# RichealYoung/BRIEF_PyTorch

Hardware: AMD Instinct MI355X
Metric: encode_voxels_per_sec (higher is better)
Workload: dtype f32; 1 GPU; SingleTask 512^3 synthetic uint16 volume, SIREN 4x256 (layers=5, features=256, w0=20), randompoint sample_size=100000, datal2, Adamax lr=1e-3; layers=5, features=256, sample_size=100000, params=198657

## Files before the change

__graft_entry__.py:

```python
import os
import subprocess
import sys

ROOT = os.path.dirname(os.path.abspath(__file__))
if ROOT not in sys.path:
    sys.path.insert(0, ROOT)


def build():
    from brief_pytorch_amd import _lib
    _lib.build(verbose=True)
    subprocess.check_call(["make", "-s", "-C", os.path.join(ROOT, "oracle")])
    import brief_pytorch_amd
    L = _lib.lib()
    for name in _lib.EXPORTS:
        assert hasattr(L, name), name
    print("build ok: libbrief_hip.so version", L.brief_version())


def smoke():
    import numpy as np
    import torch
    from brief_pytorch_amd import _lib
    from brief_pytorch_amd.networks import SIREN
    from brief_pytorch_amd.synthetic import make_volume
    from oracle import oracle as O

    assert torch.cuda.is_available(), "smoke() needs a GPU"
    _lib.lib()
    dims = (12, 16, 20)
    vol = make_volume(dims, seed=1)
    vn, side = O.normalize(vol)
    n = int(np.prod(dims))
    tv = torch.from_numpy(vn.reshape(-1, 1)).cuda()
    for layers, feats in ((5, 256), (4, 64), (3, 1100)):
        torch.manual_seed(0)
        m = SIREN(coords_channel=3, data_channel=1, features=feats, layers=layers, w0=20)
        d = O.make_desc(3, 1, layers, feats, 20.0)
        p = m.params.numpy().copy()
        m.to("cuda")
        loss, _ = m.train_step(n, tv, grid=(dims, -1.0, 1.0))
        lo, go, _, _ = O.loss_grad(d, p, O.grid_coords(dims), vn.reshape(-1, 1))
        g = m.grads.cpu().numpy()
        assert abs(loss.item() - lo) / lo < 1e-5, (loss.item(), lo)
# ... 12 lines not shown
```

brief_pytorch_amd/_lib.py:

```python
import ctypes as C
import os
import subprocess

_HERE = os.path.dirname(os.path.abspath(__file__))
LIB_PATH = os.environ.get("BRIEF_LIB", os.path.join(_HERE, "libbrief_hip.so"))
SRC = os.path.join(_HERE, "csrc", "brief_hip.hip")
_CSRC = os.path.join(_HERE, "csrc")
_DEPS = sorted(os.path.join(_CSRC, f) for f in (os.listdir(_CSRC) if os.path.isdir(_CSRC) else []) if f.endswith((".hip", ".inc", ".h"))) \
    + [os.path.join(os.path.dirname(_HERE), "include", "brief_hip.h")]
HIPCC = os.environ.get("HIPCC", "/opt/rocm/bin/hipcc")


class BriefError(RuntimeError):
    pass


class SirenDesc(C.Structure):
    _fields_ = [("cin", C.c_int32), ("cout", C.c_int32), ("layers", C.c_int32), ("features", C.c_int32),
                ("w0_first", C.c_float), ("w0_hidden", C.c_float), ("output_act", C.c_int32), ("precision", C.c_int32)]


class GridDesc(C.Structure):
    _fields_ = [("ndim", C.c_int32), ("reserved", C.c_int32), ("dims", C.c_int64 * 3), ("lo", C.c_float), ("hi", C.c_float)]

# ... 68 lines not shown

class TaperDesc(C.Structure):
    _fields_ = [("cin", C.c_int32), ("cout", C.c_int32), ("layers", C.c_int32), ("output_act", C.c_int32),
                ("widths", C.c_int32 * TAPER_MAX_LAYERS), ("w0", C.c_float * TAPER_MAX_LAYERS)]


class TaperFitJob(C.Structure):
    _fields_ = [("desc", TaperDesc)] + FitJob._fields_[1:]


FAMILIES = (("ffn", FfnDesc, FfnFitJob), ("nerf", NerfDesc, NerfFitJob), ("mfn", MfnDesc, MfnFitJob), ("taper", TaperDesc, TaperFitJob))
FAMILY_ENTRIES = ("param_count", "packed_count", "train_workspace_bytes", "repack", "forward", "forward_box", "train_step", "fit")

LOSS_KIND = {"datal2": 0, "datasmoothl1": 1, "external": 2}
OPT_KIND = {"Adamax": 0, "Adam": 1, "SGD": 2}
OUT_F32, OUT_U8, OUT_U16 = 0, 1, 2
PRECISION = {"fp32": 0, "f32": 0, "bf16": 1, "bf16x3": 2}

EXPORTS = ["brief_version", "brief_last_error", "brief_param_count", "brief_packed_count",
           "brief_train_workspace_bytes", "brief_siren_repack", "brief_siren_forward", "brief_forward_workspace_bytes", "brief_siren_forward_ws", "brief_siren_forward_box", "brief_siren_train_step", "brief_siren_fit_step",
           "brief_siren_fit", "brief_multi_fit",
           "brief_optim_step", "brief_sample_indices", "brief_sse_u16", "brief_profile_enable", "brief_profile_fused", "brief_deblock_edge", "brief_ssim_u16", "brief_ssim_partial_count",
           "brief_sincos_probe", "brief_cu_count",
           "brief_correct_chunk_elems", "brief_correct_count", "brief_correct_emit", "brief_correct_apply",
           "brief_mip_accumulate",
           "brief_quant_workspace_bytes", "brief_quant_ranges", "brief_quant_apply", "brief_quant_decode",
           "brief_siren_jac_packed_count", "brief_siren_jac_repack", "brief_siren_jac_forward", "brief_siren_jac_forward_box",
           "brief_view_clip", "brief_view_coords", "brief_view_fold", "brief_view_finish", "brief_view_sample_host", "brief_view_clip_host",
           "brief_surface_fold", "brief_surface_bracket", "brief_surface_coords", "brief_surface_step", "brief_surface_shade",
           "brief_view_sample_t_host"] \
    + ["brief_%s_%s" % (prefix, entry) for prefix, _, _ in FAMILIES for entry in FAMILY_ENTRIES]


def needs_build():
    if LIB_PATH != os.path.join(_HERE, "libbrief_hip.so"):
        return False
    if not os.path.exists(LIB_PATH):
        return True
    t = os.path.getmtime(LIB_PATH)
    return any(os.path.exists(d) and os.path.getmtime(d) > t for d in _DEPS)


DIAG_LIB_PATH = os.path.join(_HERE, "libbrief_hip_diag.so")


def build(force=False, verbose=False, diagnostics=False, defines=(), out=None):
    target = out or (DIAG_LIB_PATH if diagnostics else os.path.join(_HERE, "libbrief_hip.so"))
    if not force and not diagnostics and not defines and out is None and not needs_build():
        return LIB_PATH
    cmd = [HIPCC, "--offload-arch=gfx950", "-O3", "-std=c++17", "-ffp-contract=off", "-shared", "-fPIC", SRC, "-o", target]
    if diagnostics:
        cmd.append("-DBRIEF_DIAGNOSTICS")
    cmd += ["-D" + d for d in defines]
    if verbose:
        print(" ".join(cmd))
    subprocess.check_call(cmd)
    return target


_LIB = None


def lib():
    global _LIB
    if _LIB is not None:
        return _LIB
    import torch
    if not os.path.exists(LIB_PATH):
        raise BriefError("libbrief_hip.so is not built (run `python -c 'import __graft_entry__ as g; g.build()'`); "
                         "there is no CPU fallback for the fused SIREN path")
    L = C.CDLL(LIB_PATH)
    dp, gp, bp, vp = C.POINTER(SirenDesc), C.POINTER(GridDesc), C.POINTER(BatchDesc), C.c_void_p
    L.brief_version.restype = C.c_int
    if L.brief_version() != 130:
        raise BriefError("libbrief_hip.so is version %d, this binding needs 130 (brief_siren_forward_ws, widths to 4096): rebuild with __graft_entry__.build()" % L.brief_version())
    L.brief_last_error.restype = C.c_char_p
    L.brief_param_count.restype = C.c_int64
    L.brief_param_count.argtypes = [dp]
    L.brief_packed_count.restype = C.c_int64
    L.brief_packed_count.argtypes = [dp]
    L.brief_train_workspace_bytes.restype = C.c_int64
    L.brief_train_workspace_bytes.argtypes = [dp, C.c_int64]
# ... 83 lines not shown
```

brief_pytorch_amd/csrc/brief_hip.hip:

```cpp
#include <hip/hip_runtime.h>
#include <hip/hip_ext.h>
#include <stdint.h>
#include <stdio.h>
#include <string.h>
#include <stdlib.h>
#include <mutex>
#include "brief_layout.h"
#include "brief_math.h"

#include "brief_device.inc"
#include "brief_fused.inc"
#include "brief_lean.inc"
#include "brief_wide.inc"
#include "brief_small.inc"
#include "brief_wgrad.inc"
#include "brief_x3.inc"
#include "brief_reduce.inc"
#include "brief_bf16.inc"
#include "brief_aux.inc"
#include "brief_ffn.inc"
#include "brief_nerf.inc"
#include "brief_mfn.inc"
#include "brief_taper.inc"
#include "brief_correct.inc"
#include "brief_mip.inc"
#include "brief_quant.inc"
#include "brief_jac.inc"

static thread_local char g_err[512] = "";
static int fail(int code, const char *fmt, const char *detail = "")
{
    snprintf(g_err, sizeof(g_err), fmt, detail);
    return code;
}
#define HIP_TRY(x)                                                                  \
    do {                                                                            \
        hipError_t e_ = (x);                                                        \
        if (e_ != hipSuccess) return fail(BRIEF_ERR_LAUNCH, #x ": %s", hipGetErrorString(e_)); \
    } while (0)
// ... 46 lines not shown
static DevState *dev_state()
{
    std::lock_guard<std::recursive_mutex> lk(g_state_mu);
    static DevState *tab[kMaxDevices] = {};
    const int dev = current_device();
    if (!tab[dev]) tab[dev] = (DevState *)calloc(1, sizeof(DevState));
    return tab[dev];
}
static int dev_attr_once(const void *fn, int bytes)
{
    std::lock_guard<std::recursive_mutex> lk(g_state_mu);
    DevState *ds = dev_state();
    if (!ds) return fail(BRIEF_ERR_INVALID, "out of host memory");
    for (int i = 0; i < ds->nattr; ++i)
        if (ds->attr_fn[i] == fn && ds->attr_bytes[i] >= bytes) return 0;
    HIP_TRY(hipFuncSetAttribute(fn, hipFuncAttributeMaxDynamicSharedMemorySize, bytes));
    if (ds->nattr < 256) { ds->attr_fn[ds->nattr] = fn; ds->attr_bytes[ds->nattr] = bytes; ++ds->nattr; }
    return 0;
}

static int cu_count()
{
    static int cached[64] = {};
    int dev = 0;
    if (hipGetDevice(&dev) != hipSuccess || dev < 0 || dev >= 64) dev = 0;
    if (cached[dev] == 0) {
        int n = 0;
        if (hipDeviceGetAttribute(&n, hipDeviceAttributeMultiprocessorCount, dev) != hipSuccess || n < 1) n = 256;
        cached[dev] = n;
    }
    return cached[dev];
}
#define kCUs cu_count()
#define kWgradBlocks cu_count()

static OptimScalars optim_scalars(int kind, double lr, double beta1, double beta2, double eps, int64_t t)
{
    OptimScalars o;
    o.kind = kind;
    o.w1 = (float)(1.0 - beta1); o.fb2 = (float)beta2; o.w2 = (float)(1.0 - beta2); o.feps = (float)eps;
    o.nstep = kind == BRIEF_OPT_SGD ? (float)(-lr) : (float)(-(lr / (1.0 - pow(beta1, (double)t))));
    o.bc2s = kind == BRIEF_OPT_ADAM ? (float)sqrt(1.0 - pow(beta2, (double)t)) : 1.f;
    return o;
}

#ifdef BRIEF_DIAGNOSTICS
static const char *env_str(const char *name) { return getenv(name); }
#else
static const char *env_str(const char *) { return nullptr; }
#endif
static int env_int(const char *name, int dflt, int lo, int hi)
{
    const char *e = env_str(name);
    if (!e) return dflt;
    const int v = atoi(e);
    return v >= lo && v <= hi ? v : dflt;
}
static const int kRecWgsPerCu = 8;
static const int g_wg_per_cu = env_int("BRIEF_WG_PER_CU", BRIEF_TRAIN_WPE, 1, 4);
static const bool g_wg_per_cu_set = env_str("BRIEF_WG_PER_CU") != nullptr;
static const int g_stagger = env_int("BRIEF_STAGGER", 0, 0, 64);
static const int g_diag = env_int("BRIEF_DIAG", 0, 0, 255);
static const int g_x3_decode = env_int("BRIEF_X3_DECODE", 1, 0, 1);
static const int g_wgrad_repeat = env_int("BRIEF_WGRAD_REPEAT", 1, 1, 8);
static const int g_reduce_sg_big = env_int("BRIEF_REDUCE_SG_BIG", 4, 1, 64);
static const int g_reduce_part = env_int("BRIEF_REDUCE_PART", 0, 0, 2);
// ... 31 lines not shown
    const int64_t wgs_ = fused_wg_samples(d, train);
    const int64_t tiles = (n + wgs_ - 1) / wgs_;
    const int cap = fused_grid(d, n, train);
    FusedPlan p;
    p.grid = cap; p.pers_wgs = cap; p.pers_tiles = tiles;
    if (!train || nt > 8 || tiles <= cap || brief_use_wide(d)) return p;
    if (g_tail_rounds == 0) return p;
    int64_t rounds = tiles / cap - g_tail_rounds;
    if (rounds < 0) rounds = 0;
    const int64_t max_wgs = (int64_t)kCUs * kRecWgsPerCu;
    while (tiles - rounds * cap + (rounds ? cap : 0) > max_wgs) ++rounds;
    if (rounds * cap >= tiles) return p;
    p.pers_wgs = rounds ? cap : 0;
    p.pers_tiles = rounds * cap;
    p.grid = p.pers_wgs + (int)(tiles - p.pers_tiles);
    return p;
}
#ifndef BRIEF_WGRAD_ROUNDS
#define BRIEF_WGRAD_ROUNDS 1
#endif
#ifndef BRIEF_TAIL_PLAN
#define BRIEF_TAIL_PLAN 1
#endif
#ifndef BRIEF_TAIL_LEAN
#define BRIEF_TAIL_LEAN 0
#endif
#ifndef BRIEF_TAIL_MODE_DEFAULT
#define BRIEF_TAIL_MODE_DEFAULT 2
#endif
#ifndef BRIEF_TAIL_R
#define BRIEF_TAIL_R 1.15
#define BRIEF_TAIL_R1 1.05
#endif
#ifndef BRIEF_TAIL_MIN_SPLITS
#define BRIEF_TAIL_MIN_SPLITS 6
#endif
#ifndef BRIEF_TAIL_MIN_ROUNDS
#define BRIEF_TAIL_MIN_ROUNDS 3
#endif
struct TailPlan { int mode ; bool on; int grid_body, grid_tail; int64_t tiles_body; int ns, n_norm; int64_t kfix_n, kfix_s; };
static int wgrad_split_rule(const brief_siren_desc &d, int64_t nchunks, int min_rounds);
static const int g_tail_mode = env_int("BRIEF_TAIL_MODE", BRIEF_TAIL_MODE_DEFAULT, 0, 2);
static const int g_tail_ntmax = env_int("BRIEF_TAIL_NTMAX", 32, 9, 32);
static const int g_tail_r = env_int("BRIEF_TAIL_R", 0, 0, 1000);
static TailPlan fused_tail_plan(const brief_siren_desc &d, int64_t n)
{
    TailPlan p;
    memset(&p, 0, sizeof(p));
    if (!BRIEF_TAIL_PLAN || g_tail_mode == 0 || d.precision != BRIEF_PREC_F32 || d.layers - 2 < 1) return p;
    const int nt = brief_nt(d);
    if (nt < 8) return p;
    const int64_t tiles = (n + 31) / 32;
    const int G = fused_grid(d, n, true);
    const int64_t full = tiles / G * G, rem = tiles - full;
    if (full == 0 || rem == 0) return p;
    if (g_tail_mode == 2 && nt >= 9 && nt <= g_tail_ntmax && rem * 4 <= 3 * (int64_t)kCUs) {
        const int hidden = d.layers - 2, nq = wgrad_nq(nt), qt = (nt + nq - 1) / nq;
        const int64_t chunks = brief_npad_d(d, n) / 32, B = (int64_t)hidden * nq * nq;
        int ns = wgrad_split_rule(d, chunks, 1);
        if ((int64_t)ns * B > kCUs) ns = (int)(kCUs / B);
        const int per_xcd = kCUs / 8, tail_x = (int)((rem + 7) / 8);
        int n_norm = 0;
        if ((int64_t)ns * B <= kCUs)
            for (int c = ns - 1; c >= 1; --c) {
                const int a_ = (int)((c * B + 7) / 8), s_ = (int)(((ns - c) * B + 7) / 8);
                if (a_ + tail_x <= per_xcd && a_ + s_ <= per_xcd && (ns - c) * B >= rem) { n_norm = c; break; }
            }
        const int n_short = ns - n_norm;
        const double r = g_tail_r ? 0.01 * g_tail_r : (nt <= 16 ? BRIEF_TAIL_R : BRIEF_TAIL_R1);
        const double rho = r * 2.0 * hidden * nt * nt / (double)(qt * qt);
        const double k_norm = ((double)chunks + n_short * rho) / ns, k_short = k_norm - rho;
        if (n_norm > 0 && k_short >= 4.0 && rho < 0.8 * k_norm) {
            p.kfix_n = (int64_t)(k_norm * 65536.0); p.kfix_s = (int64_t)(k_short * 65536.0);
            const int64_t b_norm = ((int64_t)(ns - n_short) * p.kfix_n) >> 16;
            if (b_norm <= full && b_norm > 0) {
                p.mode = 2; p.on = true; p.grid_body = G; p.grid_tail = (int)rem; p.tiles_body = full; p.ns = ns; p.n_norm = ns - n_short;
                return p;
            }
        }
    }
    if (!(brief_use_wide(d) || (BRIEF_TAIL_LEAN && brief_use_lean(d, true) && nt >= 9))) return p;
    if (rem * 4 > 3 * (int64_t)G) return p;
    if (wgrad_split_rule(d, full, BRIEF_TAIL_MIN_ROUNDS) < BRIEF_TAIL_MIN_SPLITS) return p;
    p.mode = 1; p.on = true; p.grid_body = G; p.grid_tail = (int)rem; p.tiles_body = full;
    return p;
}
static int wgrad_split_rule(const brief_siren_desc &d, int64_t nchunks, int min_rounds)
{
    const int hidden = d.layers - 2;
    if (hidden <= 0) return 0;
    const int nq = wgrad_nq(brief_nt(d));
    const int64_t B = (int64_t)hidden * nq * nq;
    int64_t s = kWgradBlocks / B;
    if (s < 1) s = 1;
    if (min_rounds > 1) {
        double best = 1e30;
        for (int64_t c = 1; c <= 64; ++c) {
            const int64_t rounds = (c * B + kWgradBlocks - 1) / kWgradBlocks;
            if (rounds < min_rounds && c < 64) continue;
            const double cost = (double)rounds / (double)c + 0.0001 * (double)c;
            if (cost < best - 1e-9) { best = cost; s = c; }
        }
// ... 472 lines not shown
}

struct SmallStepPlan { FusedArgs fa; ReduceArgs ra; int grid1, nb_hidden, nb_reduce, nt, hb; };

static int launch_wgrad(const brief_siren_desc &d, const WgradArgs &wa, int blocks, hipStream_t st)
{
    const int nt = brief_nt(d);
    if (d.precision == BRIEF_PREC_BF16X3) {
        for (int rep = 0; rep < g_wgrad_repeat; ++rep)
            hipLaunchKernelGGL(k_wgrad_x3, dim3(blocks), dim3(512), sizeof(float) * wgrad_lds_floats(8), st, wa);
    } else if (nt > 8) {
        const int qt = (nt + wgrad_nq(nt) - 1) / wgrad_nq(nt);
        switch (qt) {
        case 5: hipLaunchKernelGGL((k_wgrad<0, 5>), dim3(blocks), dim3(512), sizeof(float) * wgrad_lds_floats(5), st, wa); break;
        case 6: hipLaunchKernelGGL((k_wgrad<0, 6>), dim3(blocks), dim3(512), sizeof(float) * wgrad_lds_floats(6), st, wa); break;
        case 7: hipLaunchKernelGGL((k_wgrad<0, 7>), dim3(blocks), dim3(512), sizeof(float) * wgrad_lds_floats(7), st, wa); break;
        case 8: hipLaunchKernelGGL((k_wgrad<0, 8>), dim3(blocks), dim3(512), sizeof(float) * wgrad_lds_floats(8), st, wa); break;
        default: return fail(BRIEF_ERR_INVALID, "unsupported width");
        }
    } else {
#define BRIEF_CASE(NTV)                                                                                    \
    case NTV:                                                                                              \
        hipLaunchKernelGGL((k_wgrad<NTV>), dim3(blocks), dim3(512), sizeof(float) * wgrad_lds_floats(NTV), st, wa); \
        break;
        switch (nt) {
            BRIEF_CASE(1) BRIEF_CASE(2) BRIEF_CASE(3) BRIEF_CASE(4)
            BRIEF_CASE(5) BRIEF_CASE(6) BRIEF_CASE(7) BRIEF_CASE(8)
        }
#undef BRIEF_CASE
    }
    HIP_TRY(hipGetLastError());
    return 0;
}

static int train_step_impl(const brief_siren_desc *d, const float *packed, const brief_grid_desc *grid,
                           const brief_batch_desc *batch, int loss_kind, float thr, float beta,
                           float *grads, float *loss_out, float *yhat_out,
                           void *workspace, int64_t workspace_bytes, void *stream, const UpdatePayload *upd, SmallStepPlan *plan_only = nullptr)
{
    std::lock_guard<std::recursive_mutex> state_lock(g_state_mu);
    if (int rc = check_desc(d)) return rc;
    if (int rc = check_batch(d->cin, grid, batch, true)) return rc;
    if (!packed || !grads || !loss_out || !workspace) return fail(BRIEF_ERR_INVALID, "null buffer");
    if (loss_kind < BRIEF_LOSS_L2 || loss_kind > BRIEF_LOSS_EXTERNAL) return fail(BRIEF_ERR_INVALID, "bad loss_kind");
    if (d->precision == BRIEF_PREC_BF16 ? (int64_t)32 * brief_nt(*d) * npad16(batch->n) * 2 >= ((int64_t)1 << 31)
                                       : (int64_t)32 * brief_nt(*d) * brief_npad_d(*d, batch->n) * 4 >= ((int64_t)1 << 31))
        return fail(BRIEF_ERR_INVALID, "batch too large for one train step (padded width x samples x 4 bytes must stay below 2 GiB): split it");
    const WsLayout wl = ws_layout(*d, batch->n);
    if (workspace_bytes < wl.total * (int64_t)sizeof(float)) return fail(BRIEF_ERR_WORKSPACE, "workspace too small");
    hipStream_t st = (hipStream_t)stream;
    float *ws = (float *)workspace;
    const int nt = brief_nt(*d);
    if (d->precision == BRIEF_PREC_BF16) {
        const Ws16 w16 = ws16_layout(*d, batch->n);
        const int64_t np = npad16(batch->n), FP = 32 * nt;
        const int hidden = d->layers - 2;
        const Split16 sp16 = split16(*d, batch->n);
        const int g16 = sp16.g_body + sp16.g_tail, nsp = wgrad16_splits(*d, batch->n);
        const float inv16 = (float)(1.0 / ((double)batch->n * d->cout));
        FusedArgs fa;
        memset(&fa, 0, sizeof(fa));
        fa.d = *d; fa.pk = packed;
        fa.coords = batch->coords; fa.targets = batch->targets; fa.weights = batch->weights;
        fa.idx = batch->idx; fa.offset = batch->offset; fa.n = batch->n;
        if (!batch->idx && batch->rng_pop > 0) { fa.rng_pop = (uint64_t)batch->rng_pop; fa.rng_seed = batch->rng_seed; fa.rng_step = batch->rng_step; }
        fill_grid(fa.grid, grid);
// ... 116 lines not shown
    const int64_t l0_count = (int64_t)d->features * d->cin + d->features;
    const int64_t hcount = brief_canon_head_off(*d) - l0_count;
    const int64_t skinny = d->features + (int64_t)d->cout * ((d->features + 3) / 4) + 2;
    ra.vec = (!small && g_reduce_vec && d->precision == BRIEF_PREC_F32 && rthreads * 4 <= 1024) ? (d->features % 4 == 0 ? 4 : (d->features % 2 == 0 ? 2 : 0)) : 0;
    {
        const uintptr_t bits = (uintptr_t)grads | (uintptr_t)ra.params | (uintptr_t)ra.s1 | (uintptr_t)ra.s2 | (uintptr_t)ra.pk | (uintptr_t)ra.slabs;
        while (ra.vec > 1 && bits % (sizeof(float) * ra.vec) != 0) ra.vec /= 2;
        if (ra.vec == 1) ra.vec = 0;
    }
    const int ppb = rthreads / ra.sgroups * (ra.vec ? ra.vec : 1);
    const int nb_hidden = (int)((hcount + ppb - 1) / ppb);
    const int wpb = rthreads / 64;
    const int nb_skinny = (int)((skinny + wpb - 1) / wpb);
    if (plan_only) {
        if (!small) return fail(BRIEF_ERR_INVALID, "internal: step plans exist for narrow nets only");
        plan_only->fa = fa; plan_only->ra = ra; plan_only->grid1 = grid1; plan_only->nb_hidden = nb_hidden;
        plan_only->nb_reduce = nb_hidden + nb_skinny; plan_only->nt = nt; plan_only->hb = small_hb(*d);
        return 0;
    }
    const bool prof = prof_live();
    hipEvent_t pe0 = prof ? dev_state()->prof_ev[2 * g_prof_n] : nullptr, pe1 = prof ? dev_state()->prof_ev[2 * g_prof_n + 1] : nullptr;
    if (small) {
        const int hb = small_hb(*d);
#define BRIEF_CASE(NTV, HBV)                                                                                        \
    if (nt == NTV && hb == HBV)                                                                                     \
        launch_timed(k_small<NTV, HBV>, grid1, 256, sizeof(float) * SmallLds<NTV>::TOTAL, st, fa, pe0, pe1);
        BRIEF_CASE(1, 1) BRIEF_CASE(1, 3) BRIEF_CASE(1, 5) BRIEF_CASE(1, 7)
        BRIEF_CASE(2, 1) BRIEF_CASE(2, 3) BRIEF_CASE(2, 5) BRIEF_CASE(2, 7)
#undef BRIEF_CASE
        HIP_TRY(hipGetLastError());
    } else if (!tp.on) {
        if (int rc = launch_fused<true>(fa, grid1, st, pe0, pe1)) return rc;
    }
    hipStream_t side = st;
    if (tp.on) {
        DevState *ds = dev_state();
        if (!ds) return fail(BRIEF_ERR_INVALID, "out of host memory");
        if (!ds->aux2_init) {
            HIP_TRY(hipStreamCreateWithFlags(&ds->aux2, hipStreamNonBlocking));
            HIP_TRY(hipEventCreateWithFlags(&ds->aux2_fork, hipEventDisableTiming));
            HIP_TRY(hipEventCreateWithFlags(&ds->aux2_join, hipEventDisableTiming));
            ds->aux2_init = true;
        }
        side = ds->aux2;
        fa.n_begin = 0; fa.n_end = tp.tiles_body * 32; fa.rec_base = 0;
        fa.pers_wgs = tp.grid_body; fa.pers_tiles = tp.tiles_body;
        if (int rc = launch_fused<true>(fa, tp.grid_body, st, pe0, nullptr)) return rc;
        HIP_TRY(hipEventRecord(ds->aux2_fork, st));
        HIP_TRY(hipStreamWaitEvent(side, ds->aux2_fork, 0));
        fa.n_begin = tp.tiles_body * 32; fa.n_end = 0; fa.rec_base = tp.grid_body;
        fa.pers_wgs = 0;
        if (int rc = launch_fused<true>(fa, tp.grid_tail, st, nullptr, pe1)) return rc;
    }
    if (prof) ++g_prof_n;

    if (!small && nsplit > 0) {
        WgradArgs wa;
        memset(&wa, 0, sizeof(wa));
        wa.d = *d; wa.Z = fa.Z; wa.D = fa.D; wa.npad = fa.npad; wa.nsplit = nsplit; wa.slabs = ws + wl.slabs;
        wa.stamps = ws + wl.rec + rec_region_floats(*d) - 256 * 8 * 8;
        const int per_split = (d->layers - 2) * wgrad_nq(nt) * wgrad_nq(nt);
        if (tp.mode == 2) {
            wa.uneven = 1; wa.n_norm = tp.n_norm; wa.kfix_n = tp.kfix_n; wa.kfix_s = tp.kfix_s;
            wa.kb_lo = 0; wa.kb_hi = fa.npad / 32;
            wa.split_lo = 0; wa.nsplit_here = tp.n_norm;
            if (int rc = launch_wgrad(*d, wa, wa.nsplit_here * per_split, side)) return rc;
            wa.split_lo = tp.n_norm; wa.nsplit_here = nsplit - tp.n_norm;
            if (int rc = launch_wgrad(*d, wa, wa.nsplit_here * per_split, st)) return rc;
        } else {
            const int nsA = tp.on ? nsplit - 1 : nsplit;
            wa.kb_lo = 0; wa.kb_hi = tp.on ? tp.tiles_body : fa.npad / 32; wa.split_lo = 0; wa.nsplit_here = nsA;
            for (int part = 0; part < (tp.on ? 2 : 1); ++part) {
                if (part) { wa.kb_lo = tp.tiles_body; wa.kb_hi = fa.npad / 32; wa.split_lo = nsA; wa.nsplit_here = 1; }
                if (int rc = launch_wgrad(*d, wa, wa.nsplit_here * per_split, part || !tp.on ? st : side)) return rc;
            }
        }
    }
    if (tp.on) {
        HIP_TRY(hipEventRecord(dev_state()->aux2_join, side));
        HIP_TRY(hipStreamWaitEvent(st, dev_state()->aux2_join, 0));
    }
    if (g_reduce_part == 1) hipLaunchKernelGGL(k_reduce, dim3(nb_hidden), dim3(rthreads), 0, st, ra, nb_hidden);
    else if (g_reduce_part == 2) hipLaunchKernelGGL(k_reduce, dim3(nb_skinny), dim3(rthreads), 0, st, ra, 0);
    else hipLaunchKernelGGL(k_reduce, dim3(nb_hidden + nb_skinny), dim3(rthreads), 0, st, ra, nb_hidden);
    HIP_TRY(hipGetLastError());
    return 0;
}

extern "C" {

int brief_siren_train_step(const brief_siren_desc *d, const float *packed, const brief_grid_desc *grid,
                           const brief_batch_desc *batch, int loss_kind, float thr, float beta,
                           float *grads, float *loss_out, float *yhat_out,
                           void *workspace, int64_t workspace_bytes, void *stream)
{
    return train_step_impl(d, packed, grid, batch, loss_kind, thr, beta, grads, loss_out, yhat_out, workspace, workspace_bytes,
                           stream, nullptr);
}

int brief_siren_fit_step(const brief_siren_desc *d, float *params, float *packed, const brief_grid_desc *grid,
                         const brief_batch_desc *batch, int loss_kind, float thr, float beta,
                         int optim_kind, float *state1, float *state2, double lr, double beta1, double beta2, double eps, int64_t t,
                         float *grads, float *loss_out, void *workspace, int64_t workspace_bytes, void *stream)
{
    if (optim_kind < BRIEF_OPT_ADAMAX || optim_kind > BRIEF_OPT_SGD) return fail(BRIEF_ERR_INVALID, "bad optimizer kind");
    if (!params || t < 1) return fail(BRIEF_ERR_INVALID, "bad optimizer arguments");
    if (optim_kind != BRIEF_OPT_SGD && (!state1 || !state2)) return fail(BRIEF_ERR_INVALID, "optimizer state required");
    UpdatePayload up;
    up.opt = optim_scalars(optim_kind, lr, beta1, beta2, eps, t);
    up.params = params; up.s1 = state1; up.s2 = state2; up.pk = packed;
    return train_step_impl(d, packed, grid, batch, loss_kind, thr, beta, grads, loss_out, nullptr, workspace, workspace_bytes, stream, &up);
}

static int fit_job_check(const brief_fit_job *j)
// ... 134 lines not shown
    FitGroup *groups = (FitGroup *)malloc(sizeof(FitGroup) * (size_t)njobs);
    int *unit_of = (int *)malloc(sizeof(int) * (size_t)njobs);
    double *lrs = (double *)malloc(sizeof(double) * (size_t)njobs);
    if (!groups || !unit_of || !lrs) { free(groups); free(unit_of); free(lrs); return fail(BRIEF_ERR_INVALID, "out of host memory"); }
    int ngroups = 0;
    for (int j = 0; j < njobs; ++j) {
        lrs[j] = jobs[j].lr;
        unit_of[j] = -1;
        if (!use_small(jobs[j].desc) || prof_live()) continue;
        const int nt = brief_nt(jobs[j].desc), hb = small_hb(jobs[j].desc);
        int gi = -1;
        for (int q = ngroups - 1; q >= 0; --q)
            if (groups[q].nt == nt && groups[q].hb == hb) { if (groups[q].njobs < BRIEF_GROUP_MAX) gi = q; break; }
        if (gi < 0) { gi = ngroups++; groups[gi].nt = nt; groups[gi].hb = hb; groups[gi].njobs = 0; }
        groups[gi].jobs[groups[gi].njobs++] = j;
        unit_of[j] = gi;
    }
    for (int q = 0; q < ngroups; ++q)
        if (groups[q].njobs == 1) { unit_of[groups[q].jobs[0]] = -1; groups[q].njobs = 0; }
    int nunits = 0;
    int *gslot = (int *)malloc(sizeof(int) * (size_t)(ngroups + 1));
    if (!gslot) { free(groups); free(unit_of); free(lrs); return fail(BRIEF_ERR_INVALID, "out of host memory"); }
    for (int q = 0; q < ngroups; ++q) gslot[q] = groups[q].njobs ? nunits++ : -1;
    for (int j = 0; j < njobs; ++j)
        if (unit_of[j] < 0) unit_of[j] = -1 - (nunits++);
    const int ns = nunits < kPoolStreams ? nunits : kPoolStreams;
    hipStream_t caller = (hipStream_t)stream;
    int rc = 0;
    if (hipEventRecord(g_pool_ev[kPoolStreams], caller) != hipSuccess) rc = fail(BRIEF_ERR_LAUNCH, "hipEventRecord");
    for (int s = 0; s < ns && !rc; ++s)
        if (hipStreamWaitEvent(g_pool[s], g_pool_ev[kPoolStreams], 0) != hipSuccess) rc = fail(BRIEF_ERR_LAUNCH, "hipStreamWaitEvent");
    for (int q = 0; q < ngroups && !rc; ++q)
        if (groups[q].njobs) rc = fit_group_init(groups[q], jobs, g_pool[gslot[q] % ns]);
    for (int64_t k = 0; k < steps && !rc; ++k) {
        for (int q = 0; q < ngroups && !rc; ++q)
            if (groups[q].njobs) rc = fit_group_step(groups[q], jobs, k, lrs, g_pool[gslot[q] % ns]);
        for (int j = 0; j < njobs && !rc; ++j)
            if (unit_of[j] < 0) rc = fit_job_step(&jobs[j], jobs[j].t0 + 1 + k, k, &lrs[j], g_pool[(-1 - unit_of[j]) % ns]);
    }
    for (int j = 0; j < njobs && !rc && steps > 0; ++j) {
        hipStream_t sj = g_pool[(unit_of[j] < 0 ? -1 - unit_of[j] : gslot[unit_of[j]]) % ns];
        if (jobs[j].loss_log &&
            hipMemcpyAsync(jobs[j].loss_out, jobs[j].loss_log + steps - 1, sizeof(float), hipMemcpyDeviceToDevice, sj) != hipSuccess)
            rc = fail(BRIEF_ERR_LAUNCH, "hipMemcpyAsync");
    }
    free(groups); free(unit_of); free(lrs); free(gslot);
    for (int s = 0; s < ns; ++s) {
        HIP_TRY(hipEventRecord(g_pool_ev[s], g_pool[s]));
        HIP_TRY(hipStreamWaitEvent(caller, g_pool_ev[s], 0));
    }
    return rc;
}

int brief_optim_step(int kind, float *params, const float *grads, float *state1, float *state2, int64_t count,
                     double lr, double beta1, double beta2, double eps, int64_t t, void *stream)
{
    if (kind < BRIEF_OPT_ADAMAX || kind > BRIEF_OPT_SGD) return fail(BRIEF_ERR_INVALID, "bad optimizer kind");
    if (!params || !grads || count < 1 || t < 1) return fail(BRIEF_ERR_INVALID, "bad optimizer arguments");
    if (kind != BRIEF_OPT_SGD && (!state1 || !state2)) return fail(BRIEF_ERR_INVALID, "optimizer state required");
    const OptimScalars os = optim_scalars(kind, lr, beta1, beta2, eps, t);
    hipLaunchKernelGGL(k_optim, dim3((unsigned)((count + 255) / 256)), dim3(256), 0, (hipStream_t)stream, os, params, grads,
                       state1, state2, count);
    HIP_TRY(hipGetLastError());
    return 0;
}

int brief_profile_enable(int on)
{
    std::lock_guard<std::recursive_mutex> state_lock(g_state_mu);
    DevState *ds = dev_state();
    if (!ds) return fail(BRIEF_ERR_INVALID, "out of host memory");
    if (on && !ds->prof_init) {
// ... 330 lines not shown
```

brief_pytorch_amd/csrc/brief_wgrad.inc:

```
struct WgradArgs {
    brief_siren_desc d;
    const float *Z;
    const float *D;
    int64_t npad;
    int nsplit;
    int64_t kb_lo, kb_hi;
    int split_lo, nsplit_here;
    int uneven, n_norm;
    int64_t kfix_n, kfix_s;
    float *slabs;
    float *stamps;
};

constexpr int wgrad_nq(int NT) { return (NT + 7) / 8; }
constexpr int wgrad_qt(int NT) { return (NT + wgrad_nq(NT) - 1) / wgrad_nq(NT); }
#ifndef BRIEF_WGRAD_XSPLIT
#define BRIEF_WGRAD_XSPLIT 1
#endif
#ifndef BRIEF_WGRAD_LIST
#define BRIEF_WGRAD_LIST(QT) ((QT) == 3 || (QT) == 5)
#endif
#ifndef BRIEF_WGRAD_STAGE_BIAS
#define BRIEF_WGRAD_STAGE_BIAS 1
#endif
#ifndef BRIEF_WGRAD_FRAG_PIPE
#define BRIEF_WGRAD_FRAG_PIPE 1
#endif
#ifndef BRIEF_WGRAD_FRAG_PIPE2
#define BRIEF_WGRAD_FRAG_PIPE2 1
#endif
constexpr int wgrad_wmk(int QT) { return QT >= 2 ? 2 : 1; }
constexpr int wgrad_wnk(int QT) { return QT >= 7 ? 4 : (QT >= 2 ? 2 : 1); }
constexpr bool wgrad_list(int QT) { return BRIEF_WGRAD_LIST(QT); }
constexpr int wgrad_wk(int QT) { return QT >= 7 || wgrad_list(QT) ? 1 : (QT >= 2 ? 2 : 4); }
constexpr int wgrad_lds_floats(int NT)
{
    const int QT = wgrad_qt(NT);
    const int WMk = wgrad_wmk(QT), WNk = wgrad_wnk(QT), WK = wgrad_wk(QT);
    const int NWv = WMk * WNk, TN = (QT + WNk - 1) / WNk;
    const int fold = (WK - 1) * NWv * TN * 1024 + (WK - 1) * NWv * 64, panels = 4 * 32 * QT * 36;
    return fold > panels ? fold : panels;
}

template <int NT, int QTR = 0>
__global__ __launch_bounds__(512, 2) void k_wgrad(const WgradArgs a)
{
    constexpr bool RTW = NT == 0;
    const int nt_w = RTW ? brief_nt(a.d) : NT;
    const int FP = 32 * nt_w;
    const int NQ = RTW ? (nt_w + 7) / 8 : wgrad_nq(NT);
    constexpr int QT = RTW ? QTR : wgrad_qt(NT), QP = 32 * QT;
    constexpr bool LIST = wgrad_list(QT);
    constexpr int LCNT = QT * QT / 8, LREM = QT * QT % 8;
    constexpr bool HET7 = QT == 7 && !LIST;
    constexpr bool XS = BRIEF_WGRAD_XSPLIT && (LIST || HET7) && QT * QT % 8 == 1;
    constexpr int XSLOT = LIST ? LCNT : 6;
    constexpr int WMk = HET7 || LIST ? 2 : wgrad_wmk(QT), WNk = HET7 || LIST ? 4 : wgrad_wnk(QT);
    constexpr int WK = wgrad_wk(QT);
    constexpr int NWv = WMk * WNk;
    constexpr int TM = HET7 || LIST ? 1 : (QT + WMk - 1) / WMk, TN = LIST ? LCNT + (LREM ? 1 : 0) : (HET7 ? 7 : (QT + WNk - 1) / WNk);
    constexpr bool MEX = QT % WMk == 0, NEX = QT % WNk == 0;
    constexpr int LDSW = 36;
    constexpr int NLD = (QP * 8 + 511) / 512;
    constexpr int PANEL = QP * LDSW;
    constexpr bool FULL = (QP * 8) % 512 == 0;
    extern __shared__ __attribute__((aligned(16))) float smem[];

    const int tid = threadIdx.x;
    const int lane = tid & 63;
    const int wave = __builtin_amdgcn_readfirstlane(tid >> 6);
    const int hi = lane >> 5, ln = lane & 31;
    const int wk = wave / NWv, wrem = wave % NWv;
    const int wmk = wrem / WNk, wnk = wrem % WNk;
    const bool kactive = wk < WK;
    const int quad = blockIdx.x % (NQ * NQ), bsl = blockIdx.x / (NQ * NQ);
    const int qm = quad / NQ, qn = quad % NQ;
    const bool uneven = RTW && a.uneven;
    const int hidden_l = a.d.layers - 2;
    const int l = uneven ? 1 + bsl % hidden_l : 1 + bsl / a.nsplit_here;
    const int split = uneven ? bsl / hidden_l : bsl % a.nsplit_here;
    const int64_t nchunks = a.kb_hi - a.kb_lo;
    int64_t c0 = a.kb_lo + nchunks * split / a.nsplit_here, c1 = a.kb_lo + nchunks * (split + 1) / a.nsplit_here;
    if (uneven) {
        const int g0 = a.split_lo + split, g1 = g0 + 1;
        c0 = (g0 <= a.n_norm ? g0 * a.kfix_n : a.n_norm * a.kfix_n + (g0 - a.n_norm) * a.kfix_s) >> 16;
        c1 = g1 >= a.nsplit ? a.kb_hi : ((g1 <= a.n_norm ? g1 * a.kfix_n : a.n_norm * a.kfix_n + (g1 - a.n_norm) * a.kfix_s) >> 16);
    }
    const float *Dl = a.D + (int64_t)(l - 1) * FP * a.npad + qm * QP * 32;
    const float *Zl = a.Z + (int64_t)(l - 1) * FP * a.npad + qn * QP * 32;

    f32x16 acc[TM][TN];
    float dbacc[TM];
#pragma unroll
    for (int i = 0; i < TM; ++i) {
        dbacc[i] = 0.f;
#pragma unroll
        for (int jn = 0; jn < TN; ++jn)
#pragma unroll
            for (int r = 0; r < 16; ++r) acc[i][jn][r] = 0.f;
    }
    float dbl[LIST ? TN : 1];
    int lmt[LIST ? TN : 1], lnt[LIST ? TN : 1];
    if (LIST) {
        const int first = XS ? wave * LCNT : wave * LCNT + (wave > 8 - LREM ? wave - (8 - LREM) : 0);
#pragma unroll
        for (int k = 0; k < TN; ++k) {
            const int t = first + k < QT * QT ? first + k : QT * QT - 1;
            lmt[k] = t / QT; lnt[k] = t % QT; dbl[k] = 0.f;
        }
    }
    constexpr bool SBIAS = BRIEF_WGRAD_STAGE_BIAS && QT == 8;
    const bool want_bias = SBIAS && qn == 0;
    float bsum[NLD];
#pragma unroll
    for (int i = 0; i < NLD; ++i) bsum[i] = 0.f;
    float4 ra[NLD], rb[NLD];
    const int panel_bytes = (int)((int64_t)FP * a.npad * 4) - (RTW ? 0 : (NQ - 1) * QP * 128);
    const int rows_m = RTW ? FP - qm * QP : QP, rows_n = RTW ? FP - qn * QP : QP;
    const __amdgpu_buffer_rsrc_t rsD = __builtin_amdgcn_make_buffer_rsrc((void *)Dl, 0, panel_bytes, 0x00020000);
// ... 361 lines not shown
```

Measured before the change: 101.6 million voxels/s.

## Extend uneven tail split to nt=8 with side-stream overlap and boundary-table wgrad

Turns on the mode-2 uneven tail plan for features=256 (nt=8) when the device reports 8 XCDs and 256 CUs. In that case the tail fused launch and the short wgrad splits go to a side stream, and the normal wgrad splits run on the main stream. A new wgrad variant reads precomputed K-split boundaries from a table in the kernel arguments and uses a 2D grid. The aim is to overlap the partial-wave tail of the fused forward/backward with weight-gradient work. In exchange the code gains extra stream and event handling, a larger kernel argument struct, and a parallel build of the diagnostics library.

After: 101.5 million voxels/s. About the same (-0.1%).

```diff
diff --git a/__graft_entry__.py b/__graft_entry__.py
--- a/__graft_entry__.py
+++ b/__graft_entry__.py
@@ -8,8 +8,24 @@
 
 
 def build():
+    import threading
     from brief_pytorch_amd import _lib
-    _lib.build(verbose=True)
+    errs = []
+
+    def diag():
+        try:
+            _lib.build(verbose=True, diagnostics=True)
+        except Exception as e:
+            errs.append(e)
+
+    t = threading.Thread(target=diag)
+    t.start()
+    try:
+        _lib.build(verbose=True)
+    finally:
+        t.join()
+    if errs:
+        raise errs[0]
     subprocess.check_call(["make", "-s", "-C", os.path.join(ROOT, "oracle")])
     import brief_pytorch_amd
     L = _lib.lib()
diff --git a/brief_pytorch_amd/_lib.py b/brief_pytorch_amd/_lib.py
--- a/brief_pytorch_amd/_lib.py
+++ b/brief_pytorch_amd/_lib.py
@@ -124,12 +124,14 @@
     + ["brief_%s_%s" % (prefix, entry) for prefix, _, _ in FAMILIES for entry in FAMILY_ENTRIES]
 
 
-def needs_build():
-    if LIB_PATH != os.path.join(_HERE, "libbrief_hip.so"):
-        return False
-    if not os.path.exists(LIB_PATH):
+def needs_build(target=None):
+    if target is None:
+        if LIB_PATH != os.path.join(_HERE, "libbrief_hip.so"):
+            return False
+        target = LIB_PATH
+    if not os.path.exists(target):
         return True
-    t = os.path.getmtime(LIB_PATH)
+    t = os.path.getmtime(target)
     return any(os.path.exists(d) and os.path.getmtime(d) > t for d in _DEPS)
 
 
@@ -138,8 +140,8 @@
 
 def build(force=False, verbose=False, diagnostics=False, defines=(), out=None):
     target = out or (DIAG_LIB_PATH if diagnostics else os.path.join(_HERE, "libbrief_hip.so"))
-    if not force and not diagnostics and not defines and out is None and not needs_build():
-        return LIB_PATH
+    if not force and not defines and out is None and not needs_build(DIAG_LIB_PATH if diagnostics else None):
+        return DIAG_LIB_PATH if diagnostics else LIB_PATH
     cmd = [HIPCC, "--offload-arch=gfx950", "-O3", "-std=c++17", "-ffp-contract=off", "-shared", "-fPIC", SRC, "-o", target]
     if diagnostics:
         cmd.append("-DBRIEF_DIAGNOSTICS")
diff --git a/brief_pytorch_amd/csrc/brief_hip.hip b/brief_pytorch_amd/csrc/brief_hip.hip
--- a/brief_pytorch_amd/csrc/brief_hip.hip
+++ b/brief_pytorch_amd/csrc/brief_hip.hip
@@ -5,6 +5,7 @@
 #include <string.h>
 #include <stdlib.h>
 #include <mutex>
+#include <type_traits>
 #include "brief_layout.h"
 #include "brief_math.h"
 
@@ -117,6 +118,18 @@
     return cached[dev];
 }
 #define kCUs cu_count()
+static int xcd_count()
+{
+    static int cached[64] = {};
+    int dev = 0;
+    if (hipGetDevice(&dev) != hipSuccess || dev < 0 || dev >= 64) dev = 0;
+    if (cached[dev] == 0) {
+        int n = 0;
+        if (hipDeviceGetAttribute(&n, hipDeviceAttributeNumberOfXccs, dev) != hipSuccess || n < 1) { (void)hipGetLastError(); n = -1; }
+        cached[dev] = n;
+    }
+    return cached[dev] > 0 ? cached[dev] : 0;
+}
 #define kWgradBlocks cu_count()
 
 static OptimScalars optim_scalars(int kind, double lr, double beta1, double beta2, double eps, int64_t t)
@@ -214,6 +227,12 @@
 #define BRIEF_TAIL_R 1.15
 #define BRIEF_TAIL_R1 1.05
 #endif
+#ifndef BRIEF_TAIL_NT8_DEFAULT
+#define BRIEF_TAIL_NT8_DEFAULT 1
+#endif
+#ifndef BRIEF_TAIL_R8
+#define BRIEF_TAIL_R8 1.75
+#endif
 #ifndef BRIEF_TAIL_MIN_SPLITS
 #define BRIEF_TAIL_MIN_SPLITS 6
 #endif
@@ -225,6 +244,8 @@
 static const int g_tail_mode = env_int("BRIEF_TAIL_MODE", BRIEF_TAIL_MODE_DEFAULT, 0, 2);
 static const int g_tail_ntmax = env_int("BRIEF_TAIL_NTMAX", 32, 9, 32);
 static const int g_tail_r = env_int("BRIEF_TAIL_R", 0, 0, 1000);
+static const int g_tail_nt8 = env_int("BRIEF_TAIL_NT8", BRIEF_TAIL_NT8_DEFAULT, 0, 1);
+static const int g_tail_swap = env_int("BRIEF_TAIL_SWAP", 1, 0, 1);
 static TailPlan fused_tail_plan(const brief_siren_desc &d, int64_t n)
 {
     TailPlan p;
@@ -236,20 +257,23 @@
     const int G = fused_grid(d, n, true);
     const int64_t full = tiles / G * G, rem = tiles - full;
     if (full == 0 || rem == 0) return p;
-    if (g_tail_mode == 2 && nt >= 9 && nt <= g_tail_ntmax && rem * 4 <= 3 * (int64_t)kCUs) {
+    const int xcds = xcd_count();
+    const bool nt8 = nt == 8 && g_tail_nt8 && !BRIEF_FUSED64 && !g_wg_per_cu_set && g_tail_rounds == 0 && xcds == 8 && kCUs == 8 * 32;
+    if (g_tail_mode == 2 && ((nt >= 9 && nt <= g_tail_ntmax) || nt8) && rem * 4 <= 3 * (int64_t)kCUs) {
         const int hidden = d.layers - 2, nq = wgrad_nq(nt), qt = (nt + nq - 1) / nq;
         const int64_t chunks = brief_npad_d(d, n) / 32, B = (int64_t)hidden * nq * nq;
         int ns = wgrad_split_rule(d, chunks, 1);
         if ((int64_t)ns * B > kCUs) ns = (int)(kCUs / B);
-        const int per_xcd = kCUs / 8, tail_x = (int)((rem + 7) / 8);
+        const int nx = xcds > 0 ? xcds : 8;
+        const int per_xcd = kCUs / nx, tail_x = (int)((rem + nx - 1) / nx);
         int n_norm = 0;
-        if ((int64_t)ns * B <= kCUs)
+        if ((int64_t)ns * B <= kCUs && (nt != 8 || ns <= BRIEF_WGRAD_TAB_MAX))
             for (int c = ns - 1; c >= 1; --c) {
-                const int a_ = (int)((c * B + 7) / 8), s_ = (int)(((ns - c) * B + 7) / 8);
+                const int a_ = (int)((c * B + nx - 1) / nx), s_ = (int)(((ns - c) * B + nx - 1) / nx);
                 if (a_ + tail_x <= per_xcd && a_ + s_ <= per_xcd && (ns - c) * B >= rem) { n_norm = c; break; }
             }
         const int n_short = ns - n_norm;
-        const double r = g_tail_r ? 0.01 * g_tail_r : (nt <= 16 ? BRIEF_TAIL_R : BRIEF_TAIL_R1);
+        const double r = g_tail_r ? 0.01 * g_tail_r : (nt == 8 ? BRIEF_TAIL_R8 : (nt <= 16 ? BRIEF_TAIL_R : BRIEF_TAIL_R1));
         const double rho = r * 2.0 * hidden * nt * nt / (double)(qt * qt);
         const double k_norm = ((double)chunks + n_short * rho) / ns, k_short = k_norm - rho;
         if (n_norm > 0 && k_short >= 4.0 && rho < 0.8 * k_norm) {
@@ -788,6 +812,46 @@
     HIP_TRY(hipGetLastError());
     return 0;
 }
+
+static int launch_wgrad_tab(const WgradTabArgs &wa, hipStream_t st)
+{
+    hipLaunchKernelGGL((k_wgrad<8, 0, WgradTabArgs>), dim3(wa.d.layers - 2, wa.nsplit_here), dim3(512), sizeof(float) * wgrad_lds_floats(8), st, wa);
+    HIP_TRY(hipGetLastError());
+    return 0;
+}
+
+static int g_in_pool = 0;
+static bool tail_side_stream(DevState *ds, hipStream_t st, hipStream_t *side)
+{
+    hipStreamCaptureStatus cs = hipStreamCaptureStatusNone, cs2 = hipStreamCaptureStatusNone;
+    unsigned long long id = 0, id2 = 0;
+    if (hipStreamGetCaptureInfo(st, &cs, &id) != hipSuccess) { (void)hipGetLastError(); return false; }
+    if (!ds->aux2_init) {
+        if (cs != hipStreamCaptureStatusNone) return false;
+        if (hipStreamCreateWithFlags(&ds->aux2, hipStreamNonBlocking) != hipSuccess) { (void)hipGetLastError(); return false; }
+        if (hipEventCreateWithFlags(&ds->aux2_fork, hipEventDisableTiming) != hipSuccess ||
+            hipEventCreateWithFlags(&ds->aux2_join, hipEventDisableTiming) != hipSuccess) { (void)hipGetLastError(); return false; }
+        ds->aux2_init = true;
+    }
+    if (g_in_pool) return false;
+    if (hipStreamGetCaptureInfo(ds->aux2, &cs2, &id2) != hipSuccess) { (void)hipGetLastError(); return false; }
+    if (cs2 != hipStreamCaptureStatusNone && !(cs == hipStreamCaptureStatusActive && cs2 == hipStreamCaptureStatusActive && id == id2)) return false;
+    *side = ds->aux2;
+    return true;
+}
+struct SideJoin {
+    hipStream_t st, side; hipEvent_t ev; bool open;
+    SideJoin() : st(nullptr), side(nullptr), ev(nullptr), open(false) {}
+    int join()
+    {
+        if (!open) return 0;
+        open = false;
+        HIP_TRY(hipEventRecord(ev, side));
+        HIP_TRY(hipStreamWaitEvent(st, ev, 0));
+        return 0;
+    }
+    ~SideJoin() { if (open) { (void)hipEventRecord(ev, side); (void)hipStreamWaitEvent(st, ev, 0); } }
+};
 
 static int train_step_impl(const brief_siren_desc *d, const float *packed, const brief_grid_desc *grid,
                            const brief_batch_desc *batch, int loss_kind, float thr, float beta,
@@ -970,25 +1034,30 @@
     } else if (!tp.on) {
         if (int rc = launch_fused<true>(fa, grid1, st, pe0, pe1)) return rc;
     }
-    hipStream_t side = st;
+    hipStream_t side = st, s_tail = st, s_norm = st;
+    SideJoin sj;
+    if (!small) {
+        DevState *ds = dev_state();
+        if (!ds) return fail(BRIEF_ERR_INVALID, "out of host memory");
+        hipStream_t s2 = st;
+        const bool forked = tail_side_stream(ds, st, &s2);
+        if (tp.on && forked) { side = s2; sj.st = st; sj.side = side; sj.ev = ds->aux2_join; }
+        s_norm = side;
+    }
     if (tp.on) {
         DevState *ds = dev_state();
-        if (!ds) return fail(BRIEF_ERR_INVALID, "out of host memory");
-        if (!ds->aux2_init) {
-            HIP_TRY(hipStreamCreateWithFlags(&ds->aux2, hipStreamNonBlocking));
-            HIP_TRY(hipEventCreateWithFlags(&ds->aux2_fork, hipEventDisableTiming));
-            HIP_TRY(hipEventCreateWithFlags(&ds->aux2_join, hipEventDisableTiming));
-            ds->aux2_init = true;
-        }
-        side = ds->aux2;
         fa.n_begin = 0; fa.n_end = tp.tiles_body * 32; fa.rec_base = 0;
         fa.pers_wgs = tp.grid_body; fa.pers_tiles = tp.tiles_body;
         if (int rc = launch_fused<true>(fa, tp.grid_body, st, pe0, nullptr)) return rc;
-        HIP_TRY(hipEventRecord(ds->aux2_fork, st));
-        HIP_TRY(hipStreamWaitEvent(side, ds->aux2_fork, 0));
+        if (side != st) {
+            HIP_TRY(hipEventRecord(ds->aux2_fork, st));
+            HIP_TRY(hipStreamWaitEvent(side, ds->aux2_fork, 0));
+            sj.open = true;
+        }
         fa.n_begin = tp.tiles_body * 32; fa.n_end = 0; fa.rec_base = tp.grid_body;
         fa.pers_wgs = 0;
-        if (int rc = launch_fused<true>(fa, tp.grid_tail, st, nullptr, pe1)) return rc;
+        if (nt == 8 && tp.mode == 2 && g_tail_swap) { s_tail = side; s_norm = st; }
+        if (int rc = launch_fused<true>(fa, tp.grid_tail, s_tail, nullptr, pe1)) return rc;
     }
     if (prof) ++g_prof_n;
 
@@ -1001,10 +1070,27 @@
         if (tp.mode == 2) {
             wa.uneven = 1; wa.n_norm = tp.n_norm; wa.kfix_n = tp.kfix_n; wa.kfix_s = tp.kfix_s;
             wa.kb_lo = 0; wa.kb_hi = fa.npad / 32;
-            wa.split_lo = 0; wa.nsplit_here = tp.n_norm;
-            if (int rc = launch_wgrad(*d, wa, wa.nsplit_here * per_split, side)) return rc;
-            wa.split_lo = tp.n_norm; wa.nsplit_here = nsplit - tp.n_norm;
-            if (int rc = launch_wgrad(*d, wa, wa.nsplit_here * per_split, st)) return rc;
+            if (nt == 8) {
+                WgradTabArgs wt;
+                memset(&wt, 0, sizeof(wt));
+                static_cast<WgradArgs &>(wt) = wa;
+                wt.uneven = 0;
+                if (nsplit > BRIEF_WGRAD_TAB_MAX) return fail(BRIEF_ERR_INVALID, "internal: too many K splits for the boundary table");
+                for (int g = 0; g <= nsplit; ++g) {
+                    const int64_t b = g >= nsplit ? wa.kb_hi : ((g <= tp.n_norm ? g * tp.kfix_n : tp.n_norm * tp.kfix_n + (g - tp.n_norm) * tp.kfix_s) >> 16);
+                    if (b > wa.kb_hi || (g > 0 && b <= wt.bnd[g - 1])) return fail(BRIEF_ERR_INVALID, "internal: K-split boundaries out of order");
+                    wt.bnd[g] = (int)b;
+                }
+                wt.split_lo = 0; wt.nsplit_here = tp.n_norm;
+                if (int rc = launch_wgrad_tab(wt, s_norm)) return rc;
+                wt.split_lo = tp.n_norm; wt.nsplit_here = nsplit - tp.n_norm;
+                if (int rc = launch_wgrad_tab(wt, s_tail)) return rc;
+            } else {
+                wa.split_lo = 0; wa.nsplit_here = tp.n_norm;
+                if (int rc = launch_wgrad(*d, wa, wa.nsplit_here * per_split, side)) return rc;
+                wa.split_lo = tp.n_norm; wa.nsplit_here = nsplit - tp.n_norm;
+                if (int rc = launch_wgrad(*d, wa, wa.nsplit_here * per_split, st)) return rc;
+            }
         } else {
             const int nsA = tp.on ? nsplit - 1 : nsplit;
             wa.kb_lo = 0; wa.kb_hi = tp.on ? tp.tiles_body : fa.npad / 32; wa.split_lo = 0; wa.nsplit_here = nsA;
@@ -1014,10 +1100,7 @@
             }
         }
     }
-    if (tp.on) {
-        HIP_TRY(hipEventRecord(dev_state()->aux2_join, side));
-        HIP_TRY(hipStreamWaitEvent(st, dev_state()->aux2_join, 0));
-    }
+    if (int rc = sj.join()) return rc;
     if (g_reduce_part == 1) hipLaunchKernelGGL(k_reduce, dim3(nb_hidden), dim3(rthreads), 0, st, ra, nb_hidden);
     else if (g_reduce_part == 2) hipLaunchKernelGGL(k_reduce, dim3(nb_skinny), dim3(rthreads), 0, st, ra, 0);
     else hipLaunchKernelGGL(k_reduce, dim3(nb_hidden + nb_skinny), dim3(rthreads), 0, st, ra, nb_hidden);
@@ -1218,12 +1301,14 @@
         if (hipStreamWaitEvent(g_pool[s], g_pool_ev[kPoolStreams], 0) != hipSuccess) rc = fail(BRIEF_ERR_LAUNCH, "hipStreamWaitEvent");
     for (int q = 0; q < ngroups && !rc; ++q)
         if (groups[q].njobs) rc = fit_group_init(groups[q], jobs, g_pool[gslot[q] % ns]);
+    ++g_in_pool;
     for (int64_t k = 0; k < steps && !rc; ++k) {
         for (int q = 0; q < ngroups && !rc; ++q)
             if (groups[q].njobs) rc = fit_group_step(groups[q], jobs, k, lrs, g_pool[gslot[q] % ns]);
         for (int j = 0; j < njobs && !rc; ++j)
             if (unit_of[j] < 0) rc = fit_job_step(&jobs[j], jobs[j].t0 + 1 + k, k, &lrs[j], g_pool[(-1 - unit_of[j]) % ns]);
     }
+    --g_in_pool;
     for (int j = 0; j < njobs && !rc && steps > 0; ++j) {
         hipStream_t sj = g_pool[(unit_of[j] < 0 ? -1 - unit_of[j] : gslot[unit_of[j]]) % ns];
         if (jobs[j].loss_log &&
diff --git a/brief_pytorch_amd/csrc/brief_wgrad.inc b/brief_pytorch_amd/csrc/brief_wgrad.inc
--- a/brief_pytorch_amd/csrc/brief_wgrad.inc
+++ b/brief_pytorch_amd/csrc/brief_wgrad.inc
@@ -11,6 +11,8 @@
     float *slabs;
     float *stamps;
 };
+#define BRIEF_WGRAD_TAB_MAX 256
+struct WgradTabArgs : WgradArgs { int bnd[BRIEF_WGRAD_TAB_MAX + 1]; };
 
 constexpr int wgrad_nq(int NT) { return (NT + 7) / 8; }
 constexpr int wgrad_qt(int NT) { return (NT + wgrad_nq(NT) - 1) / wgrad_nq(NT); }
@@ -42,10 +44,11 @@
     return fold > panels ? fold : panels;
 }
 
-template <int NT, int QTR = 0>
-__global__ __launch_bounds__(512, 2) void k_wgrad(const WgradArgs a)
+template <int NT, int QTR = 0, typename ArgsT = WgradArgs>
+__global__ __launch_bounds__(512, 2) void k_wgrad(const ArgsT a)
 {
     constexpr bool RTW = NT == 0;
+    constexpr bool TAB = !std::is_same<ArgsT, WgradArgs>::value;
     const int nt_w = RTW ? brief_nt(a.d) : NT;
     const int FP = 32 * nt_w;
     const int NQ = RTW ? (nt_w + 7) / 8 : wgrad_nq(NT);
@@ -73,18 +76,22 @@
     const int wk = wave / NWv, wrem = wave % NWv;
     const int wmk = wrem / WNk, wnk = wrem % WNk;
     const bool kactive = wk < WK;
-    const int quad = blockIdx.x % (NQ * NQ), bsl = blockIdx.x / (NQ * NQ);
+    const int quad = TAB ? 0 : blockIdx.x % (NQ * NQ), bsl = TAB ? 0 : blockIdx.x / (NQ * NQ);
     const int qm = quad / NQ, qn = quad % NQ;
     const bool uneven = RTW && a.uneven;
     const int hidden_l = a.d.layers - 2;
-    const int l = uneven ? 1 + bsl % hidden_l : 1 + bsl / a.nsplit_here;
-    const int split = uneven ? bsl / hidden_l : bsl % a.nsplit_here;
+    const int l = TAB ? 1 + (int)blockIdx.x : (uneven ? 1 + bsl % hidden_l : 1 + bsl / a.nsplit_here);
+    const int split = TAB ? (int)blockIdx.y : (uneven ? bsl / hidden_l : bsl % a.nsplit_here);
     const int64_t nchunks = a.kb_hi - a.kb_lo;
     int64_t c0 = a.kb_lo + nchunks * split / a.nsplit_here, c1 = a.kb_lo + nchunks * (split + 1) / a.nsplit_here;
     if (uneven) {
         const int g0 = a.split_lo + split, g1 = g0 + 1;
         c0 = (g0 <= a.n_norm ? g0 * a.kfix_n : a.n_norm * a.kfix_n + (g0 - a.n_norm) * a.kfix_s) >> 16;
         c1 = g1 >= a.nsplit ? a.kb_hi : ((g1 <= a.n_norm ? g1 * a.kfix_n : a.n_norm * a.kfix_n + (g1 - a.n_norm) * a.kfix_s) >> 16);
+    }
+    if constexpr (TAB) {
+        const int g0 = a.split_lo + split;
+        c0 = a.bnd[g0]; c1 = a.bnd[g0 + 1];
     }
     const float *Dl = a.D + (int64_t)(l - 1) * FP * a.npad + qm * QP * 32;
     const float *Zl = a.Z + (int64_t)(l - 1) * FP * a.npad + qn * QP * 32;
```
